# bioinf-mcb/Metagenomic-DeepFRI

Measured on NVIDIA B200. Metric: proteins/sec (GCN MF fwd incl. cmap), higher is better.
Workload: dtype f16 (hi/lo split weights) with f32 accumulate

## Files before the change

metagenomic-deepfri_b200/csrc/api.cu:

```cuda
#include <chrono>
#include <functional>
#include <stdarg.h>
#include <algorithm>
#include <numeric>
#include <thread>

#include "cmap_kernels.cuh"
#include "gcn.cuh"
#include "tc_engine.cuh"

namespace mdf {

static thread_local char g_err[1024] = "";

void set_error(const char *fmt, ...)
{
    va_list ap;
    va_start(ap, fmt);
    vsnprintf(g_err, sizeof g_err, fmt, ap);
    va_end(ap);
}

int head_forward(mdf_model *m, int n, const float *pooled, float *fc, float *logits, float *scores);

// ... 640 lines not shown
{
    MDF_REQUIRE(m && b && dst, "mdf_batch_fetch: bad arguments");
    mdf_ctx *ctx = m->ctx;
    MDF_CUDA(cudaSetDevice(ctx->device));
    const void *src = nullptr;
    size_t bytes = 0;
    const size_t T = (size_t)b->T;
    switch (what) {
    case 0: src = b->d_packed; bytes = (size_t)b->h_packed_off[b->n] * 4; break;
    case 1: src = b->d_deg; bytes = T * 4; break;
    case 2: src = b->tap_h[0]; bytes = T * m->H * 4; break;
    case 3: src = b->tap_h[m->n_lstm - 1]; bytes = T * m->H * 4; break;
    case 4: src = b->tap_x0; bytes = T * m->E * 4; break;
    case 5: src = b->d_pooled; bytes = (size_t)b->n * m->G * 4; break;
    case 6: src = b->tap_gc_last; bytes = T * m->gc[m->n_gc - 1] * 4; break;
    default: MDF_REQUIRE(false, "mdf_batch_fetch: unknown tap %d", what);
    }
    MDF_REQUIRE(src != nullptr, "mdf_batch_fetch: tap %d not produced by the last run", what);
    MDF_REQUIRE(dst_bytes >= bytes, "mdf_batch_fetch: destination too small (%zu < %zu)", dst_bytes, bytes);
    if (bytes) MDF_CUDA(cudaMemcpyAsync(dst, src, bytes, cudaMemcpyDeviceToHost, ctx->stream));
    MDF_CUDA(cudaStreamSynchronize(ctx->stream));
    return MDF_OK;
}

static int slot_acquire(mdf_ctx *ctx, mdf_job **out)
{
    mdf_job *sl = &ctx->slots[ctx->next_slot];
    if (sl->busy) {
        set_error("mdf_path_submit: both job slots of this context are in flight; call mdf_path_wait on the older job first");
        return MDF_EINVAL;
// ... 467 lines not shown
```

metagenomic-deepfri_b200/csrc/gcn.cuh:

```cuda
#pragma once
#include "mdf_common.cuh"

#define MDF_MAX_LSTM 4
#define MDF_MAX_GC 8

struct mdf_model {
    mdf_ctx *ctx = nullptr;
    int I = 26, H = 0, n_lstm = 0, E = 0, n_gc = 0, gc[MDF_MAX_GC] = {0}, G = 0, F = 0, C = 0;
    int act = 2;
    float alpha = 1.0f, eps = 1e-6f;
    int engine = 0;
    float *lstm_Wt[MDF_MAX_LSTM] = {nullptr};
    float *lstm_Rs[MDF_MAX_LSTM] = {nullptr};
    float *lstm_b[MDF_MAX_LSTM] = {nullptr};
    float *lstm_tab = nullptr;
    float *aa_W = nullptr, *lm_W = nullptr, *lm_b = nullptr;
    float *gc_W[MDF_MAX_GC] = {nullptr}, *gc_b[MDF_MAX_GC] = {nullptr};
    float *fc_W = nullptr, *fc_b = nullptr, *out_W = nullptr, *out_b = nullptr;
    std::vector<void *> owned;
    void *tc = nullptr;
};

struct mdf_batch {
    mdf_ctx *ctx = nullptr;
// ... 17 lines not shown
    int64_t *d_coord_off = nullptr;
    char *d_qaln = nullptr, *d_taln = nullptr;
    int64_t *d_aln_off = nullptr;
    int64_t *d_packed_off = nullptr;
    int2 *d_work = nullptr;
    int *d_order = nullptr;
    int *d_res_prot = nullptr;
    float4 *d_qc = nullptr;
    uint32_t *d_packed = nullptr;
    float *d_deg = nullptr;
    uint8_t *d_idx = nullptr;
    float *d_pooled = nullptr;
    float *d_scores = nullptr;
    float *tap_h[MDF_MAX_LSTM] = {nullptr};
    float *tap_x0 = nullptr, *tap_gc_last = nullptr;
    void *tc_meta = nullptr;
    bool reuse = false;
    bool cmap_valid = false;
    float cmap_thr2 = 0.f, cmap_eps = 0.f;
    int cmap_gen = 0;
    void *lm_cache = nullptr;
    size_t lm_cache_bytes = 0;
    unsigned long long lm_hash = 0;
};

namespace mdf {

size_t simt_workspace_bytes(const mdf_model *m, int n, int64_t T);
int simt_lstm_stack(mdf_model *m, mdf_batch *b, float **Hl, float *pre, float *Cst, unsigned *barrier);
int simt_forward(mdf_model *m, mdf_batch *b, int upto);
// ... 7 lines not shown
```

metagenomic-deepfri_b200/csrc/gcn_simt.cu:

```cuda
#include "gcn.cuh"

namespace mdf {

__constant__ int8_t c_aa_lut[256];
static bool g_lut_ready[16] = {false};

static int ensure_lut(mdf_ctx *ctx)
{
    if (ctx->device < 16 && g_lut_ready[ctx->device]) return MDF_OK;
    int8_t lut[256];
    memset(lut, -1, sizeof lut);
    const char *chars = "-DGULNTKHYWCPVSOIEFXQABZRM";
    for (int i = 0; i < 26; ++i) lut[(unsigned char)chars[i]] = (int8_t)i;
    MDF_CUDA(cudaMemcpyToSymbolAsync(c_aa_lut, lut, sizeof lut, 0, cudaMemcpyHostToDevice, ctx->stream));
    if (ctx->device < 16) g_lut_ready[ctx->device] = true;
    return MDF_OK;
}

__global__ void seq_to_idx_kernel(int64_t T, const char *__restrict__ seq, uint8_t *__restrict__ idx, int *err)
{
    int64_t i = blockIdx.x * (int64_t)blockDim.x + threadIdx.x;
    if (i >= T) return;
    int v = c_aa_lut[(unsigned char)seq[i]];
    if (v < 0) { atomicCAS(err, 0, MDF_DERR_BAD_RESIDUE); v = 0; }
// ... 409 lines not shown
    const int64_t T = b->T;
    if (n == 0) return MDF_OK;
    float *Hl[MDF_MAX_LSTM] = {nullptr}, *pre = nullptr, *Cst = nullptr, *X0 = nullptr;
    unsigned *barrier = nullptr;
    for (int l = 0; l < m->n_lstm; ++l) MDF_TRY(ctx->alloc_n(&Hl[l], (size_t)T * m->H));
    MDF_TRY(ctx->alloc_n(&pre, (size_t)T * 4 * m->H));
    MDF_TRY(ctx->alloc_n(&Cst, (size_t)n * m->H));
    MDF_TRY(ctx->alloc_n(&barrier, 256));
    MDF_TRY(ctx->alloc_n(&X0, (size_t)T * m->E));
    MDF_TRY(simt_lstm_stack(m, b, Hl, pre, Cst, barrier));
    {
        ProfScope ps(ctx, "embedding_gemm", 2.0 * T * m->H * m->E);
        Epilogue e; e.bias = m->lm_b; e.gtab = m->aa_W; e.gidx = b->d_idx; e.act = 1;
        MDF_TRY(sgemm(ctx, T, m->E, m->H, Hl[m->n_lstm - 1], m->H, m->lm_W, m->E, X0, m->E, e));
        b->tap_x0 = X0;
    }
    if (upto < 3) return MDF_OK;
    int gmax = 0;
    for (int l = 0; l < m->n_gc; ++l) gmax = gmax > m->gc[l] ? gmax : m->gc[l];
    float *Y = nullptr, *Xa = nullptr, *Xb = nullptr;
    MDF_TRY(ctx->alloc_n(&Y, (size_t)T * gmax));
    MDF_TRY(ctx->alloc_n(&Xa, (size_t)T * gmax));
    MDF_TRY(ctx->alloc_n(&Xb, (size_t)T * gmax));
    MDF_CUDA(cudaMemsetAsync(b->d_pooled, 0, (size_t)n * m->G * sizeof(float), ctx->stream));
    const float *Xin = X0;
    int kin = m->E, goff = 0;
    for (int l = 0; l < m->n_gc; ++l) {
        const int g = m->gc[l];
        {
            ProfScope ps(ctx, "graphconv_xw_gemm", 2.0 * T * kin * g);
// ... 24 lines not shown
```

metagenomic-deepfri_b200/csrc/gemm_tc.cu:

```cuda
#include <algorithm>

#include "gemm_tc.cuh"

namespace mdf {
namespace tc {

constexpr int GEMM_THREADS = 320;
__host__ __device__ constexpr int gemm_epi_warps(int epi, int bn) { return (epi == EPI_IMG_ROWSCALE && bn == 256) ? 16 : 8; }
__host__ __device__ constexpr int gemm_threads(int epi, int bn, bool expand) { return (2 + gemm_epi_warps(epi, bn) + (expand ? 4 : 0)) * 32; }

struct __align__(8) GemmBarriers {
    uint64_t full[8], empty[8], tmem_full[2], tmem_empty[2];
    uint32_t tmem_base;
};

__device__ __forceinline__ float act_f(float v, int act, float alpha)
{
    if (act == 1) return fmaxf(v, 0.0f);
    if (act == 2) return v > 0.0f ? v : alpha * (__expf(v) - 1.0f);
    return v;
}

__device__ __forceinline__ int lane_id() { return (int)(threadIdx.x & 31); }

// ... 442 lines not shown
                    for (int ta = 0; ta < a_terms; ++ta)
                        tma_tile_g2s_pair(dst + ta * TILE_BYTES, &pa.tmA[ta], ((mt * 2 + rank) * g.KB_A + kb) * (TILE_BYTES / 512), &bars.full[st]);
                    for (int tb = 0; tb < b_terms; ++tb)
                        tma_tile_g2s_pair(dst + a_bytes + tb * TILE_BYTES, &pa.tmB[tb], ((nt * 2 + rank) * g.KB_B + kb) * (TILE_BYTES / 512),
                                          &bars.full[st]);
                    if (++st == stages) { st = 0; ph ^= 1; }
                }
            }
        }
    } else if (warp == w_mma) {
        if (leader) {
            constexpr uint32_t idesc = umma_idesc_f16(256, 256);
            const uint32_t full_bar0 = pin_u32(smem_u32(&bars.full[0])), empty_bar0 = pin_u32(smem_u32(&bars.empty[0]));
            const uint32_t tfull_bar0 = pin_u32(smem_u32(&bars.tmem_full[0]));
            const uint64_t desc0 = pin_u64(umma_smem_desc(smem_u32(smem), TILE_LBO, TILE_SBO));
            int st = 0; uint32_t ph = 0;
            int acc = 0; uint32_t acc_ph = 0;
            for (int grp = pair; grp < outer; grp += n_pairs)
            for (int in = 0; in < inner; ++in) {
                mbar_wait(&bars.tmem_empty[acc], acc_ph ^ 1);
                tcgen05_fence_after();
                const uint32_t d0 = tmem_base + (uint32_t)(acc * BN);
                for (int kb = 0; kb < g.nkb; ++kb) {
                    mbar_wait1_asm(full_bar0 + 8u * st, ph);
                    const uint64_t sdesc = desc0 + (uint64_t)(st * (stage_bytes >> 4));
                    const int npairs = a_terms * b_terms;
                    for (int tp = 0; tp < npairs; ++tp) {
                        const int ta = tp / b_terms, tb = tp % b_terms;
                        const bool last = tp == npairs - 1;
                        umma_f16_pair_kblock_elect(d0, sdesc + (uint64_t)(ta * (TILE_BYTES >> 4)), sdesc + (uint64_t)((a_bytes + tb * TILE_BYTES) >> 4), idesc,
                                                   (kb | tp) ? 1u : 0u, 0u, 0u, last ? empty_bar0 + 8u * st : 0u, (uint16_t)3,
                                                   (last && kb == g.nkb - 1) ? tfull_bar0 + 8u * acc : 0u, (uint16_t)3);
                    }
                    if (++st == stages) { st = 0; ph ^= 1; }
                }
                if (++acc == 2) { acc = 0; acc_ph ^= 1; }
            }
        }
    } else {
        const int lb = (warp & 3) * 32;
        const int ch = warp >> 2;
        int acc = 0; uint32_t acc_ph = 0;
        float *cs_tab = reinterpret_cast<float *>(smem + (size_t)stages * stage_bytes);
        auto tile_nt = [&](int grp_, int in_) { return g.m_fastest ? grp_ : in_; };
        int tile_no = 0;
        const bool cg_thread = EPI == EPI_IMG_COLSCALE && g.chunk_group && threadIdx.x < BN / 32;
        if (EPI == EPI_IMG_COLSCALE && pair < outer) {
            if (threadIdx.x < BN) cs_tab[threadIdx.x] = __ldg(g.colscale + (size_t)tile_nt(pair, 0) * BN + threadIdx.x);
            if (cg_thread) reinterpret_cast<int *>(cs_tab)[BN + threadIdx.x] = __ldg(g.chunk_group + (size_t)tile_nt(pair, 0) * (BN / 32) + threadIdx.x);
            asm volatile("bar.sync 2, %0;" ::"n"(PAIR_EW * 32) : "memory");
        }
        for (int grp = pair; grp < outer; grp += n_pairs)
// ... 105 lines not shown
}

template <int EPI>
static int launch_pair(mdf_ctx *ctx, int a_terms, int b_terms, const GemmArgs &args, const size_t a_bytes[2], const size_t b_bytes[2])
{
    PairGemmArgs pa;
    memset(&pa, 0, sizeof(pa));
    pa.g = args;
    pa.a_terms = a_terms; pa.b_terms = b_terms;
    const int stage_bytes = (a_terms + b_terms) * TILE_BYTES;
    pa.stages = std::min(8, (int)((200 * 1024) / stage_bytes));
    for (int t = 0; t < a_terms; ++t) MDF_TRY(make_tile_map(&pa.tmA[t], args.A[t], a_bytes[t]));
    for (int t = 0; t < b_terms; ++t) MDF_TRY(make_tile_map(&pa.tmB[t], args.B[t], b_bytes[t]));
    size_t smem = (size_t)pa.stages * stage_bytes + 1024;
    if (EPI == EPI_IMG_COLSCALE) smem += 2 * CS_SLICE * sizeof(float);
    if (EPI == EPI_IMG_EMBED && pa.g.embed_staged) {
        const size_t tab = (size_t)EMB_ROWS * EMB_LD * sizeof(float);
        while (pa.stages > 2 && smem + tab > 226 * 1024) { --pa.stages; smem -= stage_bytes; }
        smem += tab;
    }
    auto kern = gemm_pair_kernel<EPI>;
    MDF_CUDA(cudaFuncSetAttribute(kern, cudaFuncAttributeMaxDynamicSharedMemorySize, (int)smem));
    const int outer = args.m_fastest ? args.n_tiles : args.m_tiles;
    if (outer <= 0 || args.m_tiles * args.n_tiles <= 0) return MDF_OK;
    cudaLaunchConfig_t cfg = {};
    cfg.gridDim = dim3(2 * std::min(outer, ctx->sm_count / 2));
    cfg.blockDim = dim3(PAIR_THREADS);
    cfg.dynamicSmemBytes = smem;
    cfg.stream = ctx->stream;
    cudaLaunchAttribute attr[1];
    attr[0].id = cudaLaunchAttributeClusterDimension;
    attr[0].val.clusterDim.x = 2; attr[0].val.clusterDim.y = 1; attr[0].val.clusterDim.z = 1;
    cfg.attrs = attr; cfg.numAttrs = 1;
    MDF_CUDA(cudaLaunchKernelEx(&cfg, kern, pa));
    ctx->launches++;
    return MDF_OK;
}

int launch_gemm_pair(mdf_ctx *ctx, int epi, int a_terms, int b_terms, const GemmArgs &args, const size_t a_bytes[2], const size_t b_bytes[2])
{
    if (a_terms < 1 || a_terms > 2 || b_terms < 1 || b_terms > 2 || (a_terms == 2 && b_terms == 2) || args.tile_info) {
        set_error("gemm_pair: unsupported configuration");
        return MDF_EUNSUPPORTED;
    }
    if (epi == EPI_IMG_EMBED) return launch_pair<EPI_IMG_EMBED>(ctx, a_terms, b_terms, args, a_bytes, b_bytes);
    if (epi == EPI_IMG_COLSCALE) return launch_pair<EPI_IMG_COLSCALE>(ctx, a_terms, b_terms, args, a_bytes, b_bytes);
    set_error("gemm_pair: no kernel for epilogue %d", epi);
    return MDF_EUNSUPPORTED;
}

template <int EPI, int BN>
static int launch_one(mdf_ctx *ctx, int a_terms, int b_terms, const GemmArgs &args)
{
    const int stage_bytes = (a_terms + b_terms * (BN / 128)) * TILE_BYTES;
    int stages = (int)((200 * 1024) / stage_bytes);
    if (stages > 8) stages = 8;
    if (stages < 2) { set_error("gemm_tc: stage of %d bytes does not fit twice in shared memory", stage_bytes); return MDF_EUNSUPPORTED; }
    const size_t smem = (size_t)stages * stage_bytes + 1024;
    auto kern = gemm_tc_kernel<EPI, BN>;
    MDF_CUDA(cudaFuncSetAttribute(kern, cudaFuncAttributeMaxDynamicSharedMemorySize, (int)smem));
// ... 32 lines not shown
```

metagenomic-deepfri_b200/csrc/gemm_tc.cuh:

```cuda
#pragma once
#include <cuda.h>

#include "mdf_common.cuh"
#include "tc_ptx.cuh"

namespace mdf {
namespace tc {

enum Epi : int {
    EPI_F32_BIAS = 0,
    EPI_IMG_COLSCALE,
    EPI_IMG_ROWSCALE,
    EPI_IMG_EMBED,
};

struct GemmArgs {
    const __half *A[3] = {nullptr, nullptr, nullptr};
    const __half *B[2] = {nullptr, nullptr};
    int KB_A = 0, KB_B = 0;
    int m_tiles = 0, n_tiles = 0;
    int nkb = 0;
    int m_fastest = 0;
    const int4 *tile_info = nullptr;
    float *pool = nullptr;
    int pool_ld = 0, pool_off = 0;
    long long *trace = nullptr;
    int adj_compact = 0;
    const unsigned short *adj_kb_idx = nullptr;
// ... 5 lines not shown
    __half *out_img = nullptr;
    int skip_pad_rows = 0;
    int KB_out = 0;
    const float *bias = nullptr;
    const float *rowscale = nullptr;
    const float *colscale = nullptr;
    const float *corr = nullptr;
    const int *col_group = nullptr;
    const int *chunk_group = nullptr;
    int corr_ld = 0, col_valid = 0;
    float corr_scale = 1.0f;
    const float *gtab = nullptr;
    const uint8_t *gidx = nullptr;
    int ldg = 0;
    int embed_staged = 0;
    int act = 0;
    float alpha = 1.0f;
    int m_valid = 0, n_valid = 0;
    int ablate = 0;
};

__device__ __forceinline__ uint2 adj_row_window(const uint32_t *__restrict__ row, int rw, int j0)
{
    if (j0 >= 0) {
        const int wi = j0 >> 5, sh = j0 & 31;
        const uint32_t a0 = wi < rw ? __ldg(row + wi) : 0u, a1 = wi + 1 < rw ? __ldg(row + wi + 1) : 0u, a2 = wi + 2 < rw ? __ldg(row + wi + 2) : 0u;
        return make_uint2(__funnelshift_r(a0, a1, sh), __funnelshift_r(a1, a2, sh));
    }
    const unsigned long long v = (((unsigned long long)__ldg(row + 1) << 32) | (unsigned long long)__ldg(row)) << (-j0);
    return make_uint2((uint32_t)v, (uint32_t)(v >> 32));
// ... 12 lines not shown
```

metagenomic-deepfri_b200/csrc/tc_engine.cu:

```cuda
#include <algorithm>
#include <stdlib.h>

#include "gemm_tc.cuh"
#include "lstm_fused.cuh"
#include "tc_engine.cuh"

namespace mdf {

int head_forward(mdf_model *m, int n, const float *pooled, float *fc, float *logits, float *scores);
int launch_softmax0(mdf_ctx *ctx, int64_t total, const float *logits, float *scores);

using namespace tc;

struct TcModel {
    __half *lm_W[2] = {nullptr, nullptr};
    __half *gc_W[MDF_MAX_GC][2] = {{nullptr}};
    __half *gc_dW[MDF_MAX_GC][2] = {{nullptr}};
    int xw_mean = 1;
    __half *fc_W[2] = {nullptr, nullptr};
    __half *out_W[2] = {nullptr, nullptr};
    float *out_b_pad = nullptr;
    unsigned long long lm_hash = 0;
    int head_tc = 1;
    int single_term_mask = 0;
// ... 96 lines not shown
        MDF_TRY(upload_half(m, &t->fc_W[1], lo));
        build_image_host(d->out_W, 2 * m->C, m->F, true, 2 * m->C, hi, lo, 2048.0f);
        MDF_TRY(upload_half(m, &t->out_W[0], hi));
        MDF_TRY(upload_half(m, &t->out_W[1], lo));
        std::vector<float> bp((size_t)(2 * m->C + 3) / 4 * 4, 0.0f);
        if (d->out_b) std::copy(d->out_b, d->out_b + 2 * m->C, bp.begin());
        MDF_CUDA(cudaMalloc((void **)&t->out_b_pad, bp.size() * sizeof(float)));
        m->owned.push_back(t->out_b_pad);
        MDF_CUDA(cudaMemcpy(t->out_b_pad, bp.data(), bp.size() * sizeof(float), cudaMemcpyHostToDevice));
    }
    int prev = m->E;
    for (int l = 0; l < m->n_gc; ++l) {
        build_image_host(d->gc_W[l], m->gc[l], prev, true, m->gc[l], hi, lo);
        MDF_TRY(upload_half(m, &t->gc_W[l][0], hi));
        MDF_TRY(upload_half(m, &t->gc_W[l][1], lo));
        if (l > 0 && prev % TILE_K == 0) {
            std::vector<float> dw((size_t)prev * m->gc[l]);
            for (size_t i = 0; i < dw.size(); ++i) dw[i] = (d->gc_W[l][i] - __half2float(__float2half_rn(d->gc_W[l][i]))) * 2048.0f;
            build_image_host(dw.data(), m->gc[l], prev, true, m->gc[l], hi, lo, 2048.0f);
            MDF_TRY(upload_half(m, &t->gc_dW[l][0], hi));
            MDF_TRY(upload_half(m, &t->gc_dW[l][1], lo));
        }
        prev = m->gc[l];
    }
    {
        unsigned long long hsh = 1469598103934665603ull;
        auto mix = [&](const float *p, size_t count) {
            const unsigned char *c = reinterpret_cast<const unsigned char *>(p);
            for (size_t i = 0; p && i < count * sizeof(float); ++i) { hsh ^= c[i]; hsh *= 1099511628211ull; }
        };
        for (int l = 0; l < m->n_lstm; ++l) {
// ... 64 lines not shown
    if (chunk >= total) return;
    const int64_t r = chunk / (K / 8);
    const int k = (int)(chunk % (K / 8)) * 8;
    const int s = rowmap[r];
    uint4 pk = make_uint4(0, 0, 0, 0);
    if (s >= 0) {
        const float4 a = *reinterpret_cast<const float4 *>(src + (size_t)s * K + k);
        const float4 b = *reinterpret_cast<const float4 *>(src + (size_t)s * K + k + 4);
        pk.x = pack_half2(a.x, a.y); pk.y = pack_half2(a.z, a.w);
        pk.z = pack_half2(b.x, b.y); pk.w = pack_half2(b.z, b.w);
    }
    *reinterpret_cast<uint4 *>(reinterpret_cast<uint8_t *>(img) + image_offset_bytes(r, k, KB)) = pk;
}

__global__ void image_to_f32_kernel(const __half *__restrict__ img, int K, const int *__restrict__ rowmap, int64_t Tp,
                                    float *__restrict__ dst)
{
    const int KB = K / TILE_K;
    const int64_t e = blockIdx.x * (int64_t)blockDim.x + threadIdx.x;
    if (e >= Tp * K) return;
    const int64_t r = e / K;
    const int k = (int)(e % K);
    const int s = rowmap[r];
    if (s >= 0) dst[(size_t)s * K + k] = __half2float(*reinterpret_cast<const __half *>(
                    reinterpret_cast<const uint8_t *>(img) + image_offset_bytes(r, k, KB)));
}

__global__ void pad_vectors_kernel(int64_t Tp, const int *__restrict__ rowmap, const float *__restrict__ deg,
                                   const uint8_t *__restrict__ idx, float *__restrict__ deg_pad, uint8_t *__restrict__ idx_pad)
{
    const int64_t r = blockIdx.x * (int64_t)blockDim.x + threadIdx.x;
    if (r >= Tp) return;
    const int s = rowmap[r];
    if (deg) deg_pad[r] = s >= 0 ? deg[s] : 0.0f;
    idx_pad[r] = s >= 0 ? idx[s] : (uint8_t)0;
}

__global__ void __launch_bounds__(256)
expand_adjacency_kernel(const int4 *__restrict__ tiles, const int64_t *__restrict__ seq_off,
                        const uint32_t *__restrict__ packed, const int64_t *__restrict__ packed_off,
// ... 326 lines not shown
        if (l == m->n_lstm - 1 || taps) add((size_t)Tp * m->H * 2);
    add(lstm_fused_scratch_bytes(m->ctx, m->H));
    if (taps) for (int l = 0; l < m->n_lstm; ++l) add((size_t)T * m->H * 4);
    add((size_t)Tp * 4 + (size_t)Tp / 128 * 32 + (size_t)(tiles + 1) * 16 + (size_t)(n + 1) * 8 + 2048);
    add((size_t)Tp * 4); add((size_t)Tp);
    add((size_t)(tiles + 8) * 2); add((size_t)Tp / 128 * 4);
    add((size_t)Tp * m->E * 2);
    add((size_t)Tp * gmax * 2); add((size_t)Tp * gmax * 2); add((size_t)Tp * gmax * 2);
    if (!(m->tc && static_cast<const TcModel *>(m->tc)->adj_expand)) add((size_t)tiles * TILE_BYTES + 256);
    if (taps) { add((size_t)T * gmax * 4); add((size_t)T * m->E * 4); }
    add((size_t)Tp / 32 * 4);
    for (int l = 1; l < m->n_gc; ++l) {
        add((size_t)n * gmax * 4); add((size_t)n * gmax * 4);
        for (int q = 0; q < 3; ++q) add((size_t)(cdiv(n, 128) * 128) * gmax * 2);
    }
    for (int q = 0; q < 3; ++q) add((size_t)(cdiv(n, 128) * 128) * std::max(m->G, m->F) * 2);
    add((size_t)n * m->F * 4); add((size_t)n * 2 * m->C * 4); add((size_t)n * (2 * m->C + 4) * 4);
    return b + 8192;
}

int tc_forward(mdf_model *m, mdf_batch *b, int upto, const std::function<int()> *before_graphconv)
{
    mdf_ctx *ctx = m->ctx;
    TcModel *tm = static_cast<TcModel *>(m->tc);
    const int n = b->n;
    const int64_t T = b->T;
    if (n == 0) return MDF_OK;
    cudaStream_t s = ctx->stream;

    const bool want_compact = tm->compact && tm->adj_expand && tm->adj_sparse && tm->pool_fused;
// ... 52 lines not shown
        MDF_TRY(launch_lstm_fused(ctx, m->H, n, tm->lstm_fused_W, tm->lstm_phases, tm->lstm_fused_tab, tm->lstm_fused_b2, idx_pad, b->d_order,
                                  b->d_seq_off, row_off, ctx->debug_taps ? Hlimg[0] : nullptr, Hlimg[1], scratch, b->h_order.data(),
                                  b->h_seq_off.data()));
    }
    if (b->owns_memory && b->reuse && !ctx->debug_taps) b->lm_hash = tm->lm_hash;
    if (ctx->debug_taps) {
        for (int l = 0; l < m->n_lstm; ++l) {
            float *tap = nullptr;
            MDF_TRY(ctx->alloc_n(&tap, (size_t)T * m->H));
            image_to_f32_kernel<<<(unsigned)cdiv64(Tp * m->H, 256), 256, 0, s>>>(Hlimg[l], m->H, meta->rowmap, Tp, tap);
            MDF_LAUNCH_CHECK(ctx);
            b->tap_h[l] = tap;
        }
    }
    __half *Himg = Hlimg[m->n_lstm - 1];
    {
        ProfScope ps(ctx, "embedding_gemm", 2.0 * T * m->H * m->E);
        GemmArgs g;
        g.A[0] = Himg; g.KB_A = m->H / TILE_K;
        g.B[0] = tm->lm_W[0]; g.B[1] = tm->lm_W[1]; g.KB_B = m->H / TILE_K;
        g.m_tiles = meta->m_tiles; g.n_tiles = m->E / 128; g.nkb = m->H / TILE_K;
        g.out_img = X0img; g.KB_out = m->E / TILE_K;
        g.bias = m->lm_b; g.gtab = m->aa_W; g.gidx = idx_pad; g.ldg = m->E;
        if (tm->gemm_pair && Tp % 256 == 0 && m->E % 256 == 0) {
            g.m_tiles = (int)(Tp / 256); g.n_tiles = m->E / 256;
            g.embed_staged = tm->embed_staged;
            const size_t ab[2] = {(size_t)Tp * m->H * 2, 0}, bb[2] = {(size_t)m->E * m->H * 2, (size_t)m->E * m->H * 2};
            MDF_TRY(launch_gemm_pair(ctx, EPI_IMG_EMBED, 1, (tm->single_term_mask & 1) ? 1 : 2, g, ab, bb));
        } else {
            MDF_TRY(launch_gemm_tc(ctx, EPI_IMG_EMBED, 128, 1, 2, g));
        }
    }
    b->tap_x0 = nullptr;
    if (ctx->debug_taps) {
        float *tap = nullptr;
        MDF_TRY(ctx->alloc_n(&tap, (size_t)T * m->E));
        image_to_f32_kernel<<<(unsigned)cdiv64(Tp * m->E, 256), 256, 0, s>>>(X0img, m->E, meta->rowmap, Tp, tap);
        MDF_LAUNCH_CHECK(ctx);
        b->tap_x0 = tap;
    }
    if (upto < 3) return MDF_OK;
    if (before_graphconv) {
        MDF_TRY((*before_graphconv)());
        pad_vectors_kernel<<<(unsigned)cdiv64(Tp, 256), 256, 0, s>>>(Tp, meta->rowmap, b->d_deg, b->d_idx, deg_pad, idx_pad);
        MDF_LAUNCH_CHECK(ctx);
    }
    if (meta->n_adj_tiles > 0 && !tm->adj_expand) {
        ProfScope ps(ctx, "expand_adjacency", 0.0);
        expand_adjacency_kernel<<<meta->n_adj_tiles, 256, 0, s>>>(meta->exp_tiles, b->d_seq_off, b->d_packed,
                                                                  b->d_packed_off, Aimg);
        MDF_LAUNCH_CHECK(ctx);
    }
    unsigned short *kb_idx = nullptr;
    int *kb_cnt = nullptr;
    if (tm->adj_expand && tm->adj_sparse && meta->n_adj_tiles > 0) {
        ProfScope ps(ctx, "adj_tile_scan", 0.0);
        MDF_TRY(ctx->alloc_n(&kb_idx, (size_t)meta->n_adj_tiles + 8));
        MDF_TRY(ctx->alloc_n(&kb_cnt, (size_t)meta->adj_m_tiles));
        adj_tile_scan_kernel<<<meta->adj_m_tiles, 128, 0, s>>>(meta->adj_m_tiles, meta->tile_info, b->d_packed, b->d_packed_off, b->d_seq_off,
                                                               meta->seg_off, compact ? 1 : 0, kb_idx, kb_cnt);
        MDF_LAUNCH_CHECK(ctx);
    }
    MDF_CUDA(cudaMemsetAsync(b->d_pooled, 0, (size_t)n * m->G * sizeof(float), s));
    double l2 = 0.0;
    for (int p = 0; p < n; ++p) { const double L = (double)(b->h_seq_off[p + 1] - b->h_seq_off[p]); l2 += L * L; }
    const __half *Xin = X0img;
    int kin = m->E, goff = 0;
    int *chunk_group = nullptr;
    __half *Xlast = nullptr;
    for (int l = 0; l < m->n_gc; ++l) {
        const int gd = m->gc[l];
        const bool pair_ok = tm->gemm_pair && gd % 256 == 0 && Tp % 256 == 0;
        const bool mean_corr = l > 0 && tm->xw_mean && tm->pool_fused && compact && pair_ok && tm->gc_dW[l][0] && kin % TILE_K == 0 &&
                               gd % 4 == 0 && !(tm->single_term_mask & (2 << l));
        float *corr = nullptr;
        if (mean_corr) {
            ProfScope ps(ctx, "xw_mean_corr", 2.0 * n * kin * gd);
            float *mean = nullptr;
            MDF_TRY(ctx->alloc_n(&mean, (size_t)n * kin));
            MDF_TRY(ctx->alloc_n(&corr, (size_t)n * gd));
            pool_mean_kernel<<<(unsigned)cdiv64((int64_t)n * kin, 256), 256, 0, s>>>(n, kin, b->d_pooled, m->G, goff - kin, b->d_seq_off, mean);
            MDF_LAUNCH_CHECK(ctx);
            MDF_TRY(tc_dense_split(ctx, n, mean, kin, tm->gc_dW[l], gd, gd, nullptr, 0, corr));
            if (!chunk_group) {
                MDF_TRY(ctx->alloc_n(&chunk_group, (size_t)(Tp / 32)));
                chunk_group_kernel<<<(unsigned)cdiv64(Tp / 32, 256), 256, 0, s>>>(Tp / 32, T, b->d_res_prot, chunk_group);
                MDF_LAUNCH_CHECK(ctx);
            }
        }
        {
            ProfScope ps(ctx, "graphconv_xw_gemm", 2.0 * T * kin * gd);
            GemmArgs g;
            g.A[0] = tm->gc_W[l][0]; g.A[1] = tm->gc_W[l][1]; g.KB_A = kin / TILE_K;
            g.B[0] = Xin; g.KB_B = kin / TILE_K;
            g.m_tiles = gd / 128; g.n_tiles = (int)(Tp / 256); g.nkb = kin / TILE_K;
            g.out_img = Yt; g.KB_out = (int)(Tp / TILE_K);
            g.colscale = deg_pad;
            g.m_fastest = 1;
            if (pair_ok) {
                g.m_tiles = gd / 256; g.n_tiles = (int)(Tp / 256);
                const size_t ab[2] = {(size_t)gd * kin * 2, (size_t)gd * kin * 2}, bb[2] = {(size_t)Tp * kin * 2, 0};
                if (mean_corr) { g.chunk_group = chunk_group; g.corr = corr; g.corr_ld = gd; g.corr_scale = 1.0f / 2048.0f; g.col_group = b->d_res_prot; g.col_valid = (int)T; }
                MDF_TRY(launch_gemm_pair(ctx, EPI_IMG_COLSCALE, (mean_corr || (tm->single_term_mask & (2 << l))) ? 1 : 2, 1, g, ab, bb));
            } else {
                MDF_TRY(launch_gemm_tc(ctx, EPI_IMG_COLSCALE, 256, 2, 1, g));
            }
        }
        __half *Xout = (l & 1) ? Xb : Xa;
        {
            ProfScope ps(ctx, "graphconv_adj", 2.0 * l2 * gd);
            GemmArgs g;
            g.A[0] = Aimg; g.B[0] = Yt; g.KB_B = (int)(Tp / TILE_K);
            g.tile_info = meta->tile_info;
            if (tm->adj_expand) {
                g.adj_packed = b->d_packed; g.adj_packed_off = b->d_packed_off; g.adj_seq_off = b->d_seq_off; g.adj_seg_off = meta->seg_off;
                g.adj_kb_idx = kb_idx; g.adj_kb_cnt = kb_cnt;
            }
// ... 66 lines not shown
```

metagenomic-deepfri_b200/csrc/tc_ptx.cuh:

```cuda
#pragma once
#include <cuda_fp16.h>
#include <stdint.h>

namespace mdf {
namespace tc {

__device__ __forceinline__ uint32_t smem_u32(const void *p) { return (uint32_t)__cvta_generic_to_shared(p); }

__device__ __forceinline__ bool elect_one_sync()
{
    uint32_t pred = 0;
    asm volatile(
        "{\n\t.reg .b32 rx;\n\t.reg .pred px;\n\t"
        "elect.sync rx|px, 0xffffffff;\n\t"
        "@px mov.s32 %0, 1;\n\t}"
        : "+r"(pred));
    return pred != 0;
}

__device__ __forceinline__ void st_shared_v4(uint32_t addr, uint4 v)
{
    asm volatile("st.shared.v4.b32 [%0], {%1, %2, %3, %4};" ::"r"(addr), "r"(v.x), "r"(v.y), "r"(v.z), "r"(v.w) : "memory");
}

// ... 173 lines not shown
        "elect.sync _|q, 0xffffffff;\n\t"
        "setp.ne.b32 p0, %4, 0;\n\t"
        "setp.eq.b32 pt, 0, 0;\n\t"
        "setp.ne.b32 pr, %5, 0;\n\t"
        "and.pred pr, pr, q;\n\t"
        "setp.ne.b32 pe, %7, 0;\n\t"
        "and.pred pe, pe, q;\n\t"
        "setp.ne.b32 pf, %9, 0;\n\t"
        "and.pred pf, pf, q;\n\t"
        "add.s64 a1, %1, 256;\n\t"
        "add.s64 a2, %1, 512;\n\t"
        "add.s64 a3, %1, 768;\n\t"
        "add.s64 b1, %2, 256;\n\t"
        "add.s64 b2, %2, 512;\n\t"
        "add.s64 b3, %2, 768;\n\t"
        "@pr mbarrier.arrive.expect_tx.shared::cta.b64 _, [%5], %6;\n\t"
        "@q tcgen05.mma.cta_group::2.kind::f16 [%0], %1, %2, %3, p0;\n\t"
        "@q tcgen05.mma.cta_group::2.kind::f16 [%0], a1, b1, %3, pt;\n\t"
        "@q tcgen05.mma.cta_group::2.kind::f16 [%0], a2, b2, %3, pt;\n\t"
        "@q tcgen05.mma.cta_group::2.kind::f16 [%0], a3, b3, %3, pt;\n\t"
        "@pe tcgen05.commit.cta_group::2.mbarrier::arrive::one.shared::cluster.multicast::cluster.b64 [%7], %8;\n\t"
        "@pf tcgen05.commit.cta_group::2.mbarrier::arrive::one.shared::cluster.multicast::cluster.b64 [%9], %10;\n\t}"
        ::"r"(tmem_d), "l"(a_desc), "l"(b_desc), "r"(idesc), "r"(acc_first), "r"(rearm_bar), "r"(rearm_bytes), "r"(empty_bar), "h"(empty_mask),
          "r"(free_bar), "h"(free_mask) : "memory");
}
__device__ __forceinline__ void mbar_wait2_asm(uint32_t bar_a, uint32_t parity_a, uint32_t bar_b, uint32_t parity_b)
{
    asm volatile(
        "{\n\t.reg .pred p1, p2;\n\t"
        "MDF_WAIT2:\n\t"
// ... 171 lines not shown

__device__ __forceinline__ float ex2_ftz(float x) { float y; asm("ex2.approx.ftz.f32 %0, %1;" : "=f"(y) : "f"(x)); return y; }
__device__ __forceinline__ float rcp_ftz(float x) { float y; asm("rcp.approx.ftz.f32 %0, %1;" : "=f"(y) : "f"(x)); return y; }
__device__ __forceinline__ float tanh_approx(float x) { float y; asm("tanh.approx.f32 %0, %1;" : "=f"(y) : "f"(x)); return y; }

constexpr int TILE_ROWS = 128, TILE_K = 64, TILE_BYTES = 16384;
constexpr uint32_t TILE_LBO = 2048, TILE_SBO = 128;

__host__ __device__ __forceinline__ size_t image_offset_bytes(int64_t r, int k, int KB)
{
    const int64_t rt = r >> 7;
    const int kb = k >> 6;
    return ((size_t)(rt * KB + kb)) * TILE_BYTES + (size_t)((((k & 63) >> 3) * 16 + ((r & 127) >> 3)) * 128 + (r & 7) * 16 + (k & 7) * 2);
}

__device__ __forceinline__ uint32_t pack_half2(float a, float b)
{
    __half2 h = __floats2half2_rn(a, b);
    return *reinterpret_cast<uint32_t *>(&h);
}

}
}
```

metagenomic-deepfri_b200/predict.py:

```python
from __future__ import annotations

import ctypes as C
import os
from typing import List, Optional, Sequence

import numpy as np

from . import _lib
from .batching import pack_structures, packed_offsets

_ALPHABET = b"-DGULNTKHYWCPVSOIEFXQABZRM"
_LUT = np.full(256, -1, np.int16)
_LUT[np.frombuffer(_ALPHABET, np.uint8)] = np.arange(26)


def _encode(seq: str) -> bytes:
    b = seq.encode("ascii")
    codes = _LUT[np.frombuffer(b, np.uint8)]
    bad = np.flatnonzero(codes < 0)
    if bad.size:
        raise ValueError(f"Invalid character in sequence: {seq[int(bad[0])]}")
    return b


# ... 317 lines not shown
        _lib.check(_lib.lib().mdf_path_run_stages(self._handle, batch.handle, float(threshold_sq(threshold)),
                                                  int(generated_contacts), upto))

    def fetch_scores(self, batch: PathBatch, out: Optional[np.ndarray] = None) -> np.ndarray:
        self._require_gcn("fetch_scores")
        if out is None:
            out = np.empty((batch.n, self.n_terms), np.float32)
        _lib.check(_lib.lib().mdf_batch_fetch_scores(self._handle, batch.handle, out.ctypes.data))
        return out

    def unpack_dense(self, batch: PathBatch) -> int:
        cells = C.c_int64(0)
        _lib.check(_lib.lib().mdf_batch_unpack_dense(batch.handle, None, C.byref(cells)))
        return int(cells.value)

    _TAPS = {"packed": 0, "deg": 1, "lstm1": 2, "lstm2": 3, "x0": 4, "pooled": 5, "gc_last": 6}

    def fetch(self, batch: PathBatch, what: str) -> np.ndarray:
        self._require_gcn("fetch")
        T = int(batch.seq_off[-1])
        p = self.plan
        shape, dt = {
            "packed": ((int(batch.packed_off[-1]),), np.uint32), "deg": ((T,), np.float32),
            "lstm1": ((T, p.lstm_hidden), np.float32), "lstm2": ((T, p.lstm_hidden), np.float32),
            "x0": ((T, p.lm_dim), np.float32), "pooled": ((batch.n, sum(p.gc_dims)), np.float32),
            "gc_last": ((T, p.gc_dims[-1]), np.float32)}[what]
        out = np.empty(shape, dt)
        _lib.check(_lib.lib().mdf_batch_fetch(self._handle, batch.handle, self._TAPS[what], out.ctypes.data, out.nbytes))
        return out

    def close(self):
        if getattr(self, "_handle", None):
            if getattr(self, "is_cnn", False):
                _lib.lib().mdf_cnn_model_destroy(self._handle)
            else:
                _lib.lib().mdf_model_destroy(self._handle)
            self._handle = None

    def __del__(self):
        try:
            self.close()
# ... 3 lines not shown
```

Baseline: 268,500.

## Transpose embedding GEMM with fused per-protein pooling to enable layer-0 mean correction

Adds an EMBED_T epilogue that computes the embedding GEMM transposed, with weights as the M operand and residues as N. It writes X0 in an MN-major image and accumulates per-protein column sums of X0 with atomics inside the epilogue. The pooled sum feeds the mean-correction path for the first GCN layer. That layer can then run with a single hi term plus a low-rank correction instead of two split-weight terms, using a new MN-major B descriptor MMA variant. The trade is extra atomics, a smem table stage per tile and more complex layout handling, in return for removing one full tensor-core pass in GC layer 0.

```diff
diff --git a/metagenomic-deepfri_b200/csrc/api.cu b/metagenomic-deepfri_b200/csrc/api.cu
--- a/metagenomic-deepfri_b200/csrc/api.cu
+++ b/metagenomic-deepfri_b200/csrc/api.cu
@@ -678,6 +678,7 @@
     case 4: src = b->tap_x0; bytes = T * m->E * 4; break;
     case 5: src = b->d_pooled; bytes = (size_t)b->n * m->G * 4; break;
     case 6: src = b->tap_gc_last; bytes = T * m->gc[m->n_gc - 1] * 4; break;
+    case 7: src = b->tap_x0_pool; bytes = (size_t)b->n * m->E * 4; break;
     default: MDF_REQUIRE(false, "mdf_batch_fetch: unknown tap %d", what);
     }
     MDF_REQUIRE(src != nullptr, "mdf_batch_fetch: tap %d not produced by the last run", what);
diff --git a/metagenomic-deepfri_b200/csrc/gcn.cuh b/metagenomic-deepfri_b200/csrc/gcn.cuh
--- a/metagenomic-deepfri_b200/csrc/gcn.cuh
+++ b/metagenomic-deepfri_b200/csrc/gcn.cuh
@@ -55,6 +55,7 @@
     float *d_scores = nullptr;
     float *tap_h[MDF_MAX_LSTM] = {nullptr};
     float *tap_x0 = nullptr, *tap_gc_last = nullptr;
+    float *tap_x0_pool = nullptr;
     void *tc_meta = nullptr;
     bool reuse = false;
     bool cmap_valid = false;
diff --git a/metagenomic-deepfri_b200/csrc/gcn_simt.cu b/metagenomic-deepfri_b200/csrc/gcn_simt.cu
--- a/metagenomic-deepfri_b200/csrc/gcn_simt.cu
+++ b/metagenomic-deepfri_b200/csrc/gcn_simt.cu
@@ -447,6 +447,7 @@
         Epilogue e; e.bias = m->lm_b; e.gtab = m->aa_W; e.gidx = b->d_idx; e.act = 1;
         MDF_TRY(sgemm(ctx, T, m->E, m->H, Hl[m->n_lstm - 1], m->H, m->lm_W, m->E, X0, m->E, e));
         b->tap_x0 = X0;
+        b->tap_x0_pool = nullptr;
     }
     if (upto < 3) return MDF_OK;
     int gmax = 0;
diff --git a/metagenomic-deepfri_b200/csrc/gemm_tc.cu b/metagenomic-deepfri_b200/csrc/gemm_tc.cu
--- a/metagenomic-deepfri_b200/csrc/gemm_tc.cu
+++ b/metagenomic-deepfri_b200/csrc/gemm_tc.cu
@@ -480,6 +480,7 @@
             const uint32_t full_bar0 = pin_u32(smem_u32(&bars.full[0])), empty_bar0 = pin_u32(smem_u32(&bars.empty[0]));
             const uint32_t tfull_bar0 = pin_u32(smem_u32(&bars.tmem_full[0]));
             const uint64_t desc0 = pin_u64(umma_smem_desc(smem_u32(smem), TILE_LBO, TILE_SBO));
+            const uint64_t bdesc_mn0 = EPI == EPI_IMG_COLSCALE ? umma_smem_desc(smem_u32(smem), TILE_MN_LBO, TILE_MN_SBO) : 0;
             int st = 0; uint32_t ph = 0;
             int acc = 0; uint32_t acc_ph = 0;
             for (int grp = pair; grp < outer; grp += n_pairs)
@@ -494,14 +495,92 @@
                     for (int tp = 0; tp < npairs; ++tp) {
                         const int ta = tp / b_terms, tb = tp % b_terms;
                         const bool last = tp == npairs - 1;
-                        umma_f16_pair_kblock_elect(d0, sdesc + (uint64_t)(ta * (TILE_BYTES >> 4)), sdesc + (uint64_t)((a_bytes + tb * TILE_BYTES) >> 4), idesc,
-                                                   (kb | tp) ? 1u : 0u, 0u, 0u, last ? empty_bar0 + 8u * st : 0u, (uint16_t)3,
-                                                   (last && kb == g.nkb - 1) ? tfull_bar0 + 8u * acc : 0u, (uint16_t)3);
+                        const uint64_t ad = sdesc + (uint64_t)(ta * (TILE_BYTES >> 4));
+                        const uint32_t empty_b = last ? empty_bar0 + 8u * st : 0u, full_b = (last && kb == g.nkb - 1) ? tfull_bar0 + 8u * acc : 0u;
+                        if (EPI == EPI_IMG_COLSCALE && g.b_mn_major)
+                            umma_f16_pair_kblock_mn_elect(d0, ad, bdesc_mn0 + (uint64_t)(st * (stage_bytes >> 4)) + (uint64_t)((a_bytes + tb * TILE_BYTES) >> 4),
+                                                          idesc | (1u << 16), (kb | tp) ? 1u : 0u, 0u, 0u, empty_b, (uint16_t)3, full_b, (uint16_t)3);
+                        else
+                            umma_f16_pair_kblock_elect(d0, ad, sdesc + (uint64_t)((a_bytes + tb * TILE_BYTES) >> 4), idesc,
+                                                       (kb | tp) ? 1u : 0u, 0u, 0u, empty_b, (uint16_t)3, full_b, (uint16_t)3);
                     }
                     if (++st == stages) { st = 0; ph ^= 1; }
                 }
                 if (++acc == 2) { acc = 0; acc_ph ^= 1; }
             }
+        }
+    } else if (EPI == EPI_IMG_EMBED_T) {
+        const int lb = (warp & 3) * 32;
+        const int ch = warp >> 2;
+        constexpr int CW = BN * 4 / PAIR_EW;
+        float *tab = reinterpret_cast<float *>(smem + (size_t)stages * stage_bytes);
+        int acc = 0; uint32_t acc_ph = 0;
+        for (int grp = pair; grp < outer; grp += n_pairs)
+        for (int in = 0; in < inner; ++in) {
+            const int mt = g.m_fastest ? in : grp, nt = g.m_fastest ? grp : in;
+            const int f0 = (mt * 2 + rank) * 128;
+            asm volatile("bar.sync 2, %0;" ::"n"(PAIR_EW * 32) : "memory");
+            for (int e = threadIdx.x; e < EMB_ROWS * 32; e += PAIR_EW * 32) {
+                const int row = e >> 5, c4 = (e & 31) * 4;
+                float4 w = __ldg(reinterpret_cast<const float4 *>(g.gtab + (size_t)row * g.ldg + f0 + c4));
+                if (g.bias) {
+                    const float4 bb = __ldg(reinterpret_cast<const float4 *>(g.bias + f0 + c4));
+                    w.x += bb.x; w.y += bb.y; w.z += bb.z; w.w += bb.w;
+                }
+                *reinterpret_cast<float4 *>(tab + row * 128 + c4) = w;
+            }
+            asm volatile("bar.sync 2, %0;" ::"n"(PAIR_EW * 32) : "memory");
+            const int f = f0 + lb + lane;
+            const float *tcol = tab + lb + lane;
+            uint8_t *fbase = reinterpret_cast<uint8_t *>(g.out_img) + (size_t)(f >> 6) * TILE_BYTES + (size_t)((((f & 63) >> 3) * 128) + (f & 7) * 16);
+            float psum = 0.0f;
+            int pcur = -1;
+            auto flush = [&]() { if (pcur >= 0) atomicAdd(g.pool + (size_t)pcur * g.pool_ld + f, psum); psum = 0.0f; };
+            const uint32_t trow = tmem_base + ((uint32_t)lb << 16) + (uint32_t)(acc * BN);
+            mbar_wait(&bars.tmem_full[acc], acc_ph);
+            tcgen05_fence_after();
+#pragma unroll 1
+            for (int c0 = ch * CW; c0 < (ch + 1) * CW; c0 += 32) {
+                const int n0 = nt * BN + c0;
+                const uint4 i0 = __ldg(reinterpret_cast<const uint4 *>(g.gidx + n0)), i1 = __ldg(reinterpret_cast<const uint4 *>(g.gidx + n0 + 16));
+                const int pj = n0 + lane < g.col_valid ? __ldg(g.col_group + n0 + lane) : -1;
+                uint32_t r[32];
+                tmem_ld_32x32b_x32(trow + c0, r);
+                tmem_ld_wait();
+                const uint32_t iw[8] = {i0.x, i0.y, i0.z, i0.w, i1.x, i1.y, i1.z, i1.w};
+                uint32_t pk[16];
+#pragma unroll
+                for (int q = 0; q < 16; ++q) {
+                    const int ia = (iw[q >> 1] >> (16 * (q & 1))) & 0xFF, ib = (iw[q >> 1] >> (16 * (q & 1) + 8)) & 0xFF;
+                    pk[q] = pack_half2(fmaxf(__uint_as_float(r[2 * q]) + tcol[ia * 128], 0.0f), fmaxf(__uint_as_float(r[2 * q + 1]) + tcol[ib * 128], 0.0f));
+                }
+                uint8_t *dst = fbase + (size_t)(n0 >> 7) * g.KB_out * TILE_BYTES + (size_t)(((n0 & 127) >> 3) * 1024);
+#pragma unroll
+                for (int q = 0; q < 4; ++q)
+                    *reinterpret_cast<uint4 *>(dst + q * 1024) = make_uint4(pk[4 * q], pk[4 * q + 1], pk[4 * q + 2], pk[4 * q + 3]);
+                const int p0 = __shfl_sync(0xffffffffu, pj, 0);
+                if (__all_sync(0xffffffffu, pj == p0)) {
+                    if (p0 != pcur) { flush(); pcur = p0; }
+                    float s4[4] = {0.0f, 0.0f, 0.0f, 0.0f};
+#pragma unroll
+                    for (int q = 0; q < 16; ++q) s4[q & 3] = add_f32_f16(add_f32_f16(s4[q & 3], pk[q], false), pk[q], true);
+                    psum += (s4[0] + s4[1]) + (s4[2] + s4[3]);
+                } else {
+#pragma unroll
+                    for (int j = 0; j < 32; ++j) {
+                        const int p = __shfl_sync(0xffffffffu, pj, j);
+                        if (p != pcur) { flush(); pcur = p; }
+                        psum = add_f32_f16(psum, pk[j >> 1], j & 1);
+                    }
+                }
+            }
+            flush();
+            tcgen05_fence_before();
+            __syncwarp();
+            if (lane == 0) {
+                if (leader) mbar_arrive(&bars.tmem_empty[acc]); else mbar_arrive_remote(&bars.tmem_empty[acc], 0);
+            }
+            if (++acc == 2) { acc = 0; acc_ph ^= 1; }
         }
     } else {
         const int lb = (warp & 3) * 32;
@@ -637,8 +716,8 @@
     for (int t = 0; t < b_terms; ++t) MDF_TRY(make_tile_map(&pa.tmB[t], args.B[t], b_bytes[t]));
     size_t smem = (size_t)pa.stages * stage_bytes + 1024;
     if (EPI == EPI_IMG_COLSCALE) smem += 2 * CS_SLICE * sizeof(float);
-    if (EPI == EPI_IMG_EMBED && pa.g.embed_staged) {
-        const size_t tab = (size_t)EMB_ROWS * EMB_LD * sizeof(float);
+    if ((EPI == EPI_IMG_EMBED && pa.g.embed_staged) || EPI == EPI_IMG_EMBED_T) {
+        const size_t tab = (size_t)EMB_ROWS * (EPI == EPI_IMG_EMBED_T ? 128 : EMB_LD) * sizeof(float);
         while (pa.stages > 2 && smem + tab > 226 * 1024) { --pa.stages; smem -= stage_bytes; }
         smem += tab;
     }
@@ -667,6 +746,7 @@
         return MDF_EUNSUPPORTED;
     }
     if (epi == EPI_IMG_EMBED) return launch_pair<EPI_IMG_EMBED>(ctx, a_terms, b_terms, args, a_bytes, b_bytes);
+    if (epi == EPI_IMG_EMBED_T) return launch_pair<EPI_IMG_EMBED_T>(ctx, a_terms, b_terms, args, a_bytes, b_bytes);
     if (epi == EPI_IMG_COLSCALE) return launch_pair<EPI_IMG_COLSCALE>(ctx, a_terms, b_terms, args, a_bytes, b_bytes);
     set_error("gemm_pair: no kernel for epilogue %d", epi);
     return MDF_EUNSUPPORTED;
diff --git a/metagenomic-deepfri_b200/csrc/gemm_tc.cuh b/metagenomic-deepfri_b200/csrc/gemm_tc.cuh
--- a/metagenomic-deepfri_b200/csrc/gemm_tc.cuh
+++ b/metagenomic-deepfri_b200/csrc/gemm_tc.cuh
@@ -12,6 +12,7 @@
     EPI_IMG_COLSCALE,
     EPI_IMG_ROWSCALE,
     EPI_IMG_EMBED,
+    EPI_IMG_EMBED_T,
 };
 
 struct GemmArgs {
@@ -47,6 +48,7 @@
     const uint8_t *gidx = nullptr;
     int ldg = 0;
     int embed_staged = 0;
+    int b_mn_major = 0;
     int act = 0;
     float alpha = 1.0f;
     int m_valid = 0, n_valid = 0;
diff --git a/metagenomic-deepfri_b200/csrc/tc_engine.cu b/metagenomic-deepfri_b200/csrc/tc_engine.cu
--- a/metagenomic-deepfri_b200/csrc/tc_engine.cu
+++ b/metagenomic-deepfri_b200/csrc/tc_engine.cu
@@ -134,7 +134,7 @@
         build_image_host(d->gc_W[l], m->gc[l], prev, true, m->gc[l], hi, lo);
         MDF_TRY(upload_half(m, &t->gc_W[l][0], hi));
         MDF_TRY(upload_half(m, &t->gc_W[l][1], lo));
-        if (l > 0 && prev % TILE_K == 0) {
+        if (prev % TILE_K == 0) {
             std::vector<float> dw((size_t)prev * m->gc[l]);
             for (size_t i = 0; i < dw.size(); ++i) dw[i] = (d->gc_W[l][i] - __half2float(__float2half_rn(d->gc_W[l][i]))) * 2048.0f;
             build_image_host(dw.data(), m->gc[l], prev, true, m->gc[l], hi, lo, 2048.0f);
@@ -229,7 +229,7 @@
 }
 
 __global__ void image_to_f32_kernel(const __half *__restrict__ img, int K, const int *__restrict__ rowmap, int64_t Tp,
-                                    float *__restrict__ dst)
+                                    float *__restrict__ dst, int mn_major = 0)
 {
     const int KB = K / TILE_K;
     const int64_t e = blockIdx.x * (int64_t)blockDim.x + threadIdx.x;
@@ -238,7 +238,7 @@
     const int k = (int)(e % K);
     const int s = rowmap[r];
     if (s >= 0) dst[(size_t)s * K + k] = __half2float(*reinterpret_cast<const __half *>(
-                    reinterpret_cast<const uint8_t *>(img) + image_offset_bytes(r, k, KB)));
+                    reinterpret_cast<const uint8_t *>(img) + (mn_major ? image_offset_mn_bytes(r, k, KB) : image_offset_bytes(r, k, KB))));
 }
 
 __global__ void pad_vectors_kernel(int64_t Tp, const int *__restrict__ rowmap, const float *__restrict__ deg,
@@ -595,6 +595,8 @@
         add((size_t)n * gmax * 4); add((size_t)n * gmax * 4);
         for (int q = 0; q < 3; ++q) add((size_t)(cdiv(n, 128) * 128) * gmax * 2);
     }
+    add((size_t)n * m->E * 4); add((size_t)n * m->E * 4); add((size_t)n * gmax * 4);
+    for (int q = 0; q < 3; ++q) add((size_t)(cdiv(n, 128) * 128) * m->E * 2);
     for (int q = 0; q < 3; ++q) add((size_t)(cdiv(n, 128) * 128) * std::max(m->G, m->F) * 2);
     add((size_t)n * m->F * 4); add((size_t)n * 2 * m->C * 4); add((size_t)n * (2 * m->C + 4) * 4);
     return b + 8192;
@@ -677,7 +679,30 @@
         }
     }
     __half *Himg = Hlimg[m->n_lstm - 1];
-    {
+    const bool embed_t = tm->xw_mean && tm->pool_fused && compact && tm->gemm_pair && Tp % 256 == 0 && m->E % 256 == 0 && m->gc[0] % 256 == 0 &&
+                         tm->gc_dW[0][0] && !(tm->single_term_mask & 2);
+    int *chunk_group = nullptr;
+    float *x0_pool = nullptr;
+    if (embed_t) {
+        MDF_TRY(ctx->alloc_n(&chunk_group, (size_t)(Tp / 32)));
+        chunk_group_kernel<<<(unsigned)cdiv64(Tp / 32, 256), 256, 0, s>>>(Tp / 32, T, b->d_res_prot, chunk_group);
+        MDF_LAUNCH_CHECK(ctx);
+        MDF_TRY(ctx->alloc_n(&x0_pool, (size_t)n * m->E));
+        MDF_CUDA(cudaMemsetAsync(x0_pool, 0, (size_t)n * m->E * sizeof(float), s));
+    }
+    if (embed_t) {
+        ProfScope ps(ctx, "embedding_gemm", 2.0 * T * m->H * m->E);
+        GemmArgs g;
+        g.A[0] = tm->lm_W[0]; g.A[1] = tm->lm_W[1]; g.KB_A = m->H / TILE_K;
+        g.B[0] = Himg; g.KB_B = m->H / TILE_K;
+        g.m_tiles = m->E / 256; g.n_tiles = (int)(Tp / 256); g.nkb = m->H / TILE_K;
+        g.m_fastest = 1;
+        g.out_img = X0img; g.KB_out = m->E / TILE_K;
+        g.bias = m->lm_b; g.gtab = m->aa_W; g.gidx = idx_pad; g.ldg = m->E;
+        g.pool = x0_pool; g.pool_ld = m->E; g.col_group = b->d_res_prot; g.col_valid = (int)T;
+        const size_t ab[2] = {(size_t)m->E * m->H * 2, (size_t)m->E * m->H * 2}, bb[2] = {(size_t)Tp * m->H * 2, 0};
+        MDF_TRY(launch_gemm_pair(ctx, EPI_IMG_EMBED_T, (tm->single_term_mask & 1) ? 1 : 2, 1, g, ab, bb));
+    } else {
         ProfScope ps(ctx, "embedding_gemm", 2.0 * T * m->H * m->E);
         GemmArgs g;
         g.A[0] = Himg; g.KB_A = m->H / TILE_K;
@@ -695,10 +720,11 @@
         }
     }
     b->tap_x0 = nullptr;
+    b->tap_x0_pool = ctx->debug_taps ? x0_pool : nullptr;
     if (ctx->debug_taps) {
         float *tap = nullptr;
         MDF_TRY(ctx->alloc_n(&tap, (size_t)T * m->E));
-        image_to_f32_kernel<<<(unsigned)cdiv64(Tp * m->E, 256), 256, 0, s>>>(X0img, m->E, meta->rowmap, Tp, tap);
+        image_to_f32_kernel<<<(unsigned)cdiv64(Tp * m->E, 256), 256, 0, s>>>(X0img, m->E, meta->rowmap, Tp, tap, embed_t ? 1 : 0);
         MDF_LAUNCH_CHECK(ctx);
         b->tap_x0 = tap;
     }
@@ -729,20 +755,23 @@
     for (int p = 0; p < n; ++p) { const double L = (double)(b->h_seq_off[p + 1] - b->h_seq_off[p]); l2 += L * L; }
     const __half *Xin = X0img;
     int kin = m->E, goff = 0;
-    int *chunk_group = nullptr;
     __half *Xlast = nullptr;
     for (int l = 0; l < m->n_gc; ++l) {
         const int gd = m->gc[l];
         const bool pair_ok = tm->gemm_pair && gd % 256 == 0 && Tp % 256 == 0;
-        const bool mean_corr = l > 0 && tm->xw_mean && tm->pool_fused && compact && pair_ok && tm->gc_dW[l][0] && kin % TILE_K == 0 &&
-                               gd % 4 == 0 && !(tm->single_term_mask & (2 << l));
+        const bool mean_corr = l == 0 ? embed_t
+                                      : tm->xw_mean && tm->pool_fused && compact && pair_ok && tm->gc_dW[l][0] && kin % TILE_K == 0 &&
+                                            gd % 4 == 0 && !(tm->single_term_mask & (2 << l));
         float *corr = nullptr;
         if (mean_corr) {
             ProfScope ps(ctx, "xw_mean_corr", 2.0 * n * kin * gd);
             float *mean = nullptr;
             MDF_TRY(ctx->alloc_n(&mean, (size_t)n * kin));
             MDF_TRY(ctx->alloc_n(&corr, (size_t)n * gd));
-            pool_mean_kernel<<<(unsigned)cdiv64((int64_t)n * kin, 256), 256, 0, s>>>(n, kin, b->d_pooled, m->G, goff - kin, b->d_seq_off, mean);
+            if (l == 0)
+                pool_mean_kernel<<<(unsigned)cdiv64((int64_t)n * kin, 256), 256, 0, s>>>(n, kin, x0_pool, m->E, 0, b->d_seq_off, mean);
+            else
+                pool_mean_kernel<<<(unsigned)cdiv64((int64_t)n * kin, 256), 256, 0, s>>>(n, kin, b->d_pooled, m->G, goff - kin, b->d_seq_off, mean);
             MDF_LAUNCH_CHECK(ctx);
             MDF_TRY(tc_dense_split(ctx, n, mean, kin, tm->gc_dW[l], gd, gd, nullptr, 0, corr));
             if (!chunk_group) {
@@ -764,6 +793,7 @@
                 g.m_tiles = gd / 256; g.n_tiles = (int)(Tp / 256);
                 const size_t ab[2] = {(size_t)gd * kin * 2, (size_t)gd * kin * 2}, bb[2] = {(size_t)Tp * kin * 2, 0};
                 if (mean_corr) { g.chunk_group = chunk_group; g.corr = corr; g.corr_ld = gd; g.corr_scale = 1.0f / 2048.0f; g.col_group = b->d_res_prot; g.col_valid = (int)T; }
+                g.b_mn_major = l == 0 && embed_t;
                 MDF_TRY(launch_gemm_pair(ctx, EPI_IMG_COLSCALE, (mean_corr || (tm->single_term_mask & (2 << l))) ? 1 : 2, 1, g, ab, bb));
             } else {
                 MDF_TRY(launch_gemm_tc(ctx, EPI_IMG_COLSCALE, 256, 2, 1, g));
diff --git a/metagenomic-deepfri_b200/csrc/tc_ptx.cuh b/metagenomic-deepfri_b200/csrc/tc_ptx.cuh
--- a/metagenomic-deepfri_b200/csrc/tc_ptx.cuh
+++ b/metagenomic-deepfri_b200/csrc/tc_ptx.cuh
@@ -211,6 +211,38 @@
         "add.s64 b1, %2, 256;\n\t"
         "add.s64 b2, %2, 512;\n\t"
         "add.s64 b3, %2, 768;\n\t"
+        "@pr mbarrier.arrive.expect_tx.shared::cta.b64 _, [%5], %6;\n\t"
+        "@q tcgen05.mma.cta_group::2.kind::f16 [%0], %1, %2, %3, p0;\n\t"
+        "@q tcgen05.mma.cta_group::2.kind::f16 [%0], a1, b1, %3, pt;\n\t"
+        "@q tcgen05.mma.cta_group::2.kind::f16 [%0], a2, b2, %3, pt;\n\t"
+        "@q tcgen05.mma.cta_group::2.kind::f16 [%0], a3, b3, %3, pt;\n\t"
+        "@pe tcgen05.commit.cta_group::2.mbarrier::arrive::one.shared::cluster.multicast::cluster.b64 [%7], %8;\n\t"
+        "@pf tcgen05.commit.cta_group::2.mbarrier::arrive::one.shared::cluster.multicast::cluster.b64 [%9], %10;\n\t}"
+        ::"r"(tmem_d), "l"(a_desc), "l"(b_desc), "r"(idesc), "r"(acc_first), "r"(rearm_bar), "r"(rearm_bytes), "r"(empty_bar), "h"(empty_mask),
+          "r"(free_bar), "h"(free_mask) : "memory");
+}
+__device__ __forceinline__ void umma_f16_pair_kblock_mn_elect(uint32_t tmem_d, uint64_t a_desc, uint64_t b_desc, uint32_t idesc, uint32_t acc_first,
+                                                              uint32_t rearm_bar, uint32_t rearm_bytes, uint32_t empty_bar, uint16_t empty_mask,
+                                                              uint32_t free_bar, uint16_t free_mask)
+{
+    asm volatile(
+        "{\n\t.reg .pred q, p0, pt, pr, pe, pf;\n\t"
+        ".reg .b64 a1, a2, a3, b1, b2, b3;\n\t"
+        "elect.sync _|q, 0xffffffff;\n\t"
+        "setp.ne.b32 p0, %4, 0;\n\t"
+        "setp.eq.b32 pt, 0, 0;\n\t"
+        "setp.ne.b32 pr, %5, 0;\n\t"
+        "and.pred pr, pr, q;\n\t"
+        "setp.ne.b32 pe, %7, 0;\n\t"
+        "and.pred pe, pe, q;\n\t"
+        "setp.ne.b32 pf, %9, 0;\n\t"
+        "and.pred pf, pf, q;\n\t"
+        "add.s64 a1, %1, 256;\n\t"
+        "add.s64 a2, %1, 512;\n\t"
+        "add.s64 a3, %1, 768;\n\t"
+        "add.s64 b1, %2, 16;\n\t"
+        "add.s64 b2, %2, 32;\n\t"
+        "add.s64 b3, %2, 48;\n\t"
         "@pr mbarrier.arrive.expect_tx.shared::cta.b64 _, [%5], %6;\n\t"
         "@q tcgen05.mma.cta_group::2.kind::f16 [%0], %1, %2, %3, p0;\n\t"
         "@q tcgen05.mma.cta_group::2.kind::f16 [%0], a1, b1, %3, pt;\n\t"
@@ -412,6 +444,22 @@
     return ((size_t)(rt * KB + kb)) * TILE_BYTES + (size_t)((((k & 63) >> 3) * 16 + ((r & 127) >> 3)) * 128 + (r & 7) * 16 + (k & 7) * 2);
 }
 
+constexpr uint32_t TILE_MN_LBO = 128, TILE_MN_SBO = 1024;
+
+__host__ __device__ __forceinline__ size_t image_offset_mn_bytes(int64_t r, int k, int KB)
+{
+    const int64_t rt = r >> 7;
+    const int kb = k >> 6;
+    return ((size_t)(rt * KB + kb)) * TILE_BYTES + (size_t)(((((int)r & 127) >> 3) * 8 + ((k & 63) >> 3)) * 128 + (k & 7) * 16 + (r & 7) * 2);
+}
+
+__device__ __forceinline__ float add_f32_f16(float acc, uint32_t pk, bool hi)
+{
+    const unsigned short h = hi ? (unsigned short)(pk >> 16) : (unsigned short)(pk & 0xFFFFu);
+    asm("add.rn.f32.f16 %0, %1, %0;" : "+f"(acc) : "h"(h));
+    return acc;
+}
+
 __device__ __forceinline__ uint32_t pack_half2(float a, float b)
 {
     __half2 h = __floats2half2_rn(a, b);
diff --git a/metagenomic-deepfri_b200/predict.py b/metagenomic-deepfri_b200/predict.py
--- a/metagenomic-deepfri_b200/predict.py
+++ b/metagenomic-deepfri_b200/predict.py
@@ -355,7 +355,7 @@
         _lib.check(_lib.lib().mdf_batch_unpack_dense(batch.handle, None, C.byref(cells)))
         return int(cells.value)
 
-    _TAPS = {"packed": 0, "deg": 1, "lstm1": 2, "lstm2": 3, "x0": 4, "pooled": 5, "gc_last": 6}
+    _TAPS = {"packed": 0, "deg": 1, "lstm1": 2, "lstm2": 3, "x0": 4, "pooled": 5, "gc_last": 6, "x0_pool": 7}
 
     def fetch(self, batch: PathBatch, what: str) -> np.ndarray:
         self._require_gcn("fetch")
@@ -365,7 +365,7 @@
             "packed": ((int(batch.packed_off[-1]),), np.uint32), "deg": ((T,), np.float32),
             "lstm1": ((T, p.lstm_hidden), np.float32), "lstm2": ((T, p.lstm_hidden), np.float32),
             "x0": ((T, p.lm_dim), np.float32), "pooled": ((batch.n, sum(p.gc_dims)), np.float32),
-            "gc_last": ((T, p.gc_dims[-1]), np.float32)}[what]
+            "gc_last": ((T, p.gc_dims[-1]), np.float32), "x0_pool": ((batch.n, p.lm_dim), np.float32)}[what]
         out = np.empty(shape, dt)
         _lib.check(_lib.lib().mdf_batch_fetch(self._handle, batch.handle, self._TAPS[what], out.ctypes.data, out.nbytes))
         return out
```

Result: faster. 275,200, median of 6 (+2.5%).
